# vasabi-root/gaus-slam

Measured on AMD Instinct MI355X. Metric: fwd+bwd frames/sec @ 640x480, 500k Gaussians, higher is better.
Workload: dtype f32

## Files before the change

### gaus_slam_amd/_lib.py

```python
import ctypes as C
import os

from . import _host, build as _build

ALLOC_FN = _host.ALLOC_FN

EXPORTS = ["gs2d_forward", "gs2d_backward", "gs2d_forward_posed", "gs2d_backward_posed", "gs2d_mark_visible", "sknn_dist2", "gs2d_geometry_bytes",
           "gs2d_image_bytes", "gs2d_binning_bytes", "gs2d_geometry_layout", "gs2d_binning_layout",
           "gs2d_image_layout", "gs2d_last_error", "gs2d_build_info", "gs2d_stage_timing_enable",
           "gs2d_stage_timing_read", "gs2d_slam_loss", "gs2d_adam_step", "gs2d_pose_quat", "gs2d_backward_staged", "gs2d_set_deterministic",
           "gs2d_get_deterministic", "gs2d_set_reference_binning", "gs2d_get_reference_binning", "gs2d_set_launch_ahead", "gs2d_get_launch_ahead", "gs2d_forward_batch",
           "gs2d_backward_batch", "gs2d_stage_timing_read_abs"]
MAX_FRAMES = 8


class FrameIO(C.Structure):
    _fields_ = [("geometry_alloc", ALLOC_FN), ("geometry_user", C.c_void_p), ("binning_alloc", ALLOC_FN),
                ("binning_user", C.c_void_p), ("image_alloc", ALLOC_FN), ("image_user", C.c_void_p),
                ("viewmatrix", C.c_void_p), ("projmatrix", C.c_void_p), ("cam_pos", C.c_void_p),
                ("out_color", C.c_void_p), ("out_others", C.c_void_p), ("radii", C.c_void_p)]


class FrameGrad(C.Structure):
    _fields_ = [("viewmatrix", C.c_void_p), ("projmatrix", C.c_void_p), ("campos", C.c_void_p), ("tan_fovx", C.c_float),
                ("tan_fovy", C.c_float), ("radii", C.c_void_p), ("geom_buffer", C.c_void_p), ("binning_buffer", C.c_void_p),
                ("img_buffer", C.c_void_p), ("num_rendered", C.c_int), ("dL_dpix", C.c_void_p), ("dL_depths", C.c_void_p),
                ("dL_dmean2D", C.c_void_p), ("dL_dnormal", C.c_void_p), ("dL_dopacity", C.c_void_p), ("dL_dcolor", C.c_void_p),
# ... 27 lines not shown
    L.gs2d_backward_posed.restype = i
    L.gs2d_backward_posed.argtypes = L.gs2d_backward.argtypes[:-1] + [vp, vp, vp, vp]
    L.gs2d_backward_staged.restype = i
    L.gs2d_backward_staged.argtypes = [i, i, i] + L.gs2d_backward_posed.argtypes
    L.gs2d_forward_batch.restype = i
    L.gs2d_forward_batch.argtypes = [i, C.POINTER(FrameIO), i, i, i, vp, i, i, vp, vp, vp, vp, vp, f, vp, vp, i, i,
                                     C.POINTER(C.c_int), vp]
    L.gs2d_backward_batch.restype = i
    L.gs2d_backward_batch.argtypes = [i, C.POINTER(FrameGrad), i, i, i, i, vp, i, i, vp, vp, vp, vp, f, vp, vp, i, i, vp]
    L.gs2d_pose_quat.restype = i
    L.gs2d_pose_quat.argtypes = [vp, vp, vp]
    L.gs2d_mark_visible.restype = i
    L.gs2d_mark_visible.argtypes = [i, vp, vp, vp, vp, vp]
    L.sknn_dist2.restype = i
    L.sknn_dist2.argtypes = [i, vp, vp, ALLOC_FN, vp, vp]
    for n in ("gs2d_geometry_bytes", "gs2d_binning_bytes"):
        getattr(L, n).restype = sz
        getattr(L, n).argtypes = [i]
    L.gs2d_image_bytes.restype = sz
    L.gs2d_image_bytes.argtypes = [i, i]
    L.gs2d_geometry_layout.argtypes = [i, C.POINTER(sz)]
    L.gs2d_binning_layout.argtypes = [i, C.POINTER(sz)]
    L.gs2d_image_layout.argtypes = [i, i, C.POINTER(sz)]
    L.gs2d_slam_loss.restype = i
    L.gs2d_slam_loss.argtypes = [i, i, i, vp, vp, vp, vp, f, f, f, f, f, i, i, f, f, f, vp, vp, vp, vp, vp, vp]
    L.gs2d_adam_step.restype = i
    L.gs2d_adam_step.argtypes = [i, vp, vp, C.c_double, C.c_double, f, i, C.c_ulonglong, vp, vp, vp, vp, vp]
    L.gs2d_set_deterministic.argtypes = [i]
    L.gs2d_get_deterministic.restype = i
    L.gs2d_set_reference_binning.argtypes = [i]
    L.gs2d_set_launch_ahead.argtypes = [i]
# ... 29 lines not shown
```

### gaus_slam_amd/csrc/gs2d_api.hip

```cpp
#include "gs2d_common.h"
#include "../../include/gs2d_rasterizer.h"

#include <stdio.h>
#include <stdlib.h>
#include <string.h>
#include <chrono>
#include <string>
#include <atomic>
#include <mutex>
#include <thread>
#if defined(__x86_64__) || defined(__i386__)
#include <immintrin.h>
#endif

namespace {

thread_local std::string g_err;

int fail(const char* what, hipError_t e)
{
    char buf[512];
    snprintf(buf, sizeof(buf), "gs2d: %s: %s", what, hipGetErrorString(e));
    g_err = buf;
    return -1;
// ... 162 lines not shown

size_t gs2d_geometry_bytes(int P) { return geom_layout(P).total; }
size_t gs2d_image_bytes(int width, int height) { return img_layout(width, height).total; }
size_t gs2d_binning_bytes(int R) { return bin_layout(R, g_deterministic.load() != 0).total; }

void gs2d_geometry_layout(int P, size_t o[5])
{
    const GeomLayout L = geom_layout(P);
    o[0] = L.depths; o[1] = L.tiles_touched; o[2] = L.point_offsets; o[3] = L.rec; o[4] = L.clamped;
}
void gs2d_binning_layout(int R, size_t o[2])
{
    const BinLayout L = bin_layout(R);
    o[0] = L.point_list; o[1] = L.keys;
}
void gs2d_image_layout(int width, int height, size_t o[2])
{
    const ImgLayout L = img_layout(width, height);
    o[0] = L.ranges; o[1] = L.pix;
}

}

namespace {

struct FwdShared {
    int P, D, M, width, height, use_sa, debug;
    const float* background;
    const float *means3D, *shs, *colors_precomp, *opacities, *scales, *rotations, *transMat_precomp;
    float scale_modifier;
// ... 171 lines not shown
            uint2* ranges = (uint2*)(img + IL.ranges);
            const int tile_bits = (int)higher_msb((uint32_t)(cam.gx * cam.gy));
            g_timer.begin(ST_SORT, s);
            gs2d::launch_bin_by_tile_dev(db, IL.tiles, tile_bits, ranges, s);
            const long long Rg = same_shape ? (long long)last.R : (long long)C0;
            const int cap_class = gs2d::tile_sort_capacity(Rg, IL.tiles);
            f.sort_cap = gs2d::gs2d_fused_sort_cap(cap_class);
            f.fused_sort = f.sort_cap > 0;
            if (!f.fused_sort) gs2d::launch_tile_depth_sort_dev(db, IL.tiles, ranges, cap_class, 0, s);
            g_timer.end(ST_SORT, s);
            GS2D_STAGE("bin by tile (count on the device)");
            f.ahead = true; f.cap = C0; f.det = false;
            f.bin = bin_pre;
            f.bf.ranges = ranges; f.bf.point_list = nullptr; f.bf.rec = (const float4*)(geom + GL.rec);
            f.bf.out_color = f.out_color; f.bf.out_others = f.out_others; f.bf.pix_state = (float*)(img + IL.pix);
            f.bf.hits = nullptr; f.bf.hits4 = nullptr; f.bf.zero = (float4*)(geom + GL.grad_rec);
            f.bf.keys = nullptr; f.bf.keys_alt = nullptr; f.bf.vals_alt = nullptr;
            f.bf.dev = db;
            return 0;
        }
    }
    if (!wait_total(f, s)) return fail_msg("num_rendered read-back failed");
    if (debug) GS2D_CHECK(hipStreamSynchronize(s), f.spec ? "duplicate" : "scan");
    const uint32_t num_rendered_u = *f.pinned;
    if (num_rendered_u == 0xFFFFFFFFu) return fail_msg("num_rendered read-back failed");
    if (num_rendered_u > 0x7fffffffu) return fail_msg("num_rendered overflows int32");
    const int R = (int)num_rendered_u;
    f.R = R;

    last.P = P; last.W = width; last.H = height; last.R = num_rendered_u;
    const bool reuse_pre = bin_pre && R <= C0;
// ... 39 lines not shown
        g_timer.begin(ST_RANGES, s);
        gs2d::launch_tile_ranges(R, keys, ranges, IL.tiles, s);
        g_timer.end(ST_RANGES, s);
        GS2D_STAGE("ranges");
    }
    f.sort_cap = one_pass && R > 0 ? gs2d::gs2d_fused_sort_cap(gs2d::tile_sort_capacity(R, IL.tiles)) : 0;
    f.fused_sort = f.sort_cap > 0;
    if (R > 0) {
        if (!f.fused_sort)
            gs2d::launch_tile_depth_sort(R, IL.tiles, ranges, keys, point_list, keys_alt, vals_alt, one_pass ? 1 : 0, debug ? 1 : 0, s);
        g_timer.end(ST_SORT, s);
        GS2D_STAGE("tile depth sort");
    }
    f.bf.ranges = ranges; f.bf.point_list = point_list; f.bf.rec = (const float4*)(geom + GL.rec);
    f.bf.out_color = f.out_color; f.bf.out_others = f.out_others; f.bf.pix_state = (float*)(img + IL.pix);
    f.bf.hits = (uint8_t*)(bin + BL.hits); f.bf.hits4 = (uint8_t*)(bin + BL.hits4);
    f.bf.zero = (float4*)(geom + GL.grad_rec);
    f.bf.keys = keys; f.bf.keys_alt = keys_alt; f.bf.vals_alt = vals_alt;
    f.bf.dev = gs2d::DevBin{nullptr, nullptr, 0u, 0};
    return 0;
}

int fwd_batch_fused(const FwdShared& c, FwdFrame* f, int K)
{
    const int debug = c.debug;
    hipStream_t s = c.s;
    const int P = c.P, width = c.width, height = c.height;
    const GeomLayout GL = geom_layout(P);
    const ImgLayout IL = img_layout(width, height);
    gs2d::PreFwdFrames pre;
    gs2d::BinFrames bin;
// ... 84 lines not shown
        f[k].bin_bytes = BL.total;
        gs2d::BinFrame& b = bin.f[k];
        b.capacity = (uint32_t)cap[k];
        b.total_host = nullptr;
        b.R = R;
        b.point_list = (uint32_t*)(bn + BL.point_list);
        b.keys = (uint64_t*)(bn + BL.keys);
        b.vals_alt = (uint32_t*)(bn + BL.vals_alt);
        b.keys_alt = (uint64_t*)(bn + BL.keys_alt);
        b.keys_unsorted = b.keys_alt; b.vals_unsorted = b.vals_alt;
        b.hist = (uint32_t*)(bn + BL.hist);
        b.ranges = (uint2*)(f[k].img + IL.ranges);
        gs2d::BlendFwdFrame& o = f[k].bf;
        o.ranges = b.ranges; o.point_list = b.point_list; o.rec = (const float4*)(f[k].geom + GL.rec);
        o.out_color = f[k].out_color; o.out_others = f[k].out_others; o.pix_state = (float*)(f[k].img + IL.pix);
        o.hits = (uint8_t*)(bn + BL.hits); o.hits4 = (uint8_t*)(bn + BL.hits4);
        o.zero = (float4*)(f[k].geom + GL.grad_rec);
        o.keys = b.keys; o.keys_alt = b.keys_alt; o.vals_alt = b.vals_alt;
        o.dev = gs2d::DevBin{nullptr, nullptr, 0u, 0};
    }
    if (debug) GS2D_CHECK(hipStreamSynchronize(s), "duplicate (batch)");
    for (int k = K; k < GS2D_MAX_BATCH; k++) bin.f[k] = bin.f[0];
    if (redo) {
        gs2d::launch_duplicate_batch(P, K, cam0.gx, bin, s);
        GS2D_STAGE("duplicate (batch, second launch)");
    }
    long long max_R = 0;
    bool any_empty = false;
    for (int k = 0; k < K; k++) { max_R = f[k].R > max_R ? f[k].R : max_R; any_empty = any_empty || f[k].R == 0; }
    const int sort_cap = any_empty ? 0 : gs2d::gs2d_fused_sort_cap(gs2d::tile_sort_capacity(max_R, IL.tiles));
    const bool fused_sort = sort_cap > 0;
// ... 195 lines not shown
    const bool pose_fast = (stages & 3) == 3 && g_begin == 0 && g_end == P && pose_Rt != nullptr && dL_dmean3D == nullptr && dL_dtransMat == nullptr &&
                           dL_dnormal == nullptr && dL_dsh == nullptr && shs == nullptr && scales != nullptr &&
                           rotations != nullptr && !det && !live_det;
    if (dL_dpose != nullptr && (stages & 1) != 0 && (R <= 0 || det))
        GS2D_CHECK(hipMemsetAsync(dL_dpose, 0, sizeof(float) * pose_floats, s), "memset dL_dpose");
    const GeomLayout GL = geom_layout(P);
    const BinLayout BL = bin_layout(R, det);
    if (known && (stages & 1) != 0 && R > 0 && BL.total > fr.bin_bytes)
        return fail_msg("binning chunk is smaller than the layout of this backward");
    const ImgLayout IL = img_layout(width, height);
    const float4* rec = (const float4*)(geom_buffer + GL.rec);
    const uint8_t* clamped = (const uint8_t*)(geom_buffer + GL.clamped);
    float* grad_rec = (float*)(geom_buffer + GL.grad_rec);
    const uint32_t* point_list = (const uint32_t*)(binning_buffer + BL.point_list);
    const uint8_t* hits = (const uint8_t*)(binning_buffer + BL.hits4);
    const uint2* ranges = (const uint2*)(img_buffer + IL.ranges);
    const float* pix_state = (const float*)(img_buffer + IL.pix);

    if ((stages & 1) != 0 && !det) {
        if (!(known && fr.clean))
            GS2D_CHECK(hipMemsetAsync(grad_rec, 0, sizeof(float) * GS2D_GRAD_FLOATS * (size_t)P, s), "memset grad_rec");
        if (R > 0) {
            g_timer.begin(ST_BLEND_BWD, s);
            const gs2d::BlendBwdFrame bf = {ranges, point_list, rec, pix_state, hits, dL_dpix, dL_depths, grad_rec, nullptr,
                                            (const uint16_t*)(binning_buffer + BL.hits), pose_fast ? grad_rec + 4 * (size_t)P : nullptr};
            gs2d::launch_blend_bwd(width, height, 1, &bf, background, use_sa, dL_dpose, pose_floats, s);
            g_timer.end(ST_BLEND_BWD, s);
            GS2D_STAGE("blend_bwd");
        }
    }
    if ((stages & 1) != 0 && det) {
        float* det_slots = (float*)(binning_buffer + BL.det_slots);
        uint32_t* det_inv = (uint32_t*)(binning_buffer + BL.det_inv);
        g_timer.begin(ST_BLEND_BWD, s);
        if (R > 0) {
            GS2D_CHECK(hipMemsetAsync(det_slots, 0, sizeof(float) * GS2D_GRAD_FLOATS * 4 * (size_t)R, s), "memset det_slots");
            const gs2d::BlendBwdFrame bf = {ranges, point_list, rec, pix_state, hits, dL_dpix, dL_depths, grad_rec, det_slots,
                                            (const uint16_t*)(binning_buffer + BL.hits), nullptr};
            gs2d::launch_blend_bwd(width, height, 1, &bf, background, use_sa, nullptr, 0, s);
        }
        gs2d::launch_det_reduce(P, R, width, height, ranges, point_list, (const ushort4*)(geom_buffer + GL.rect),
                                (const uint32_t*)(geom_buffer + GL.tiles_touched),
                                (const uint32_t*)(geom_buffer + GL.point_offsets), hits, det_inv, det_slots, grad_rec, s);
        g_timer.end(ST_BLEND_BWD, s);
        GS2D_STAGE("blend_bwd (deterministic)");
    }
    if ((stages & 2) != 0 && g_end > g_begin) {
        const float focal_y = height / (2.0f * tan_fovy);
        const float focal_x = width / (2.0f * tan_fovx);
        CamParams cam;
        cam.vm = viewmatrix; cam.pm = projmatrix; cam.campos = campos;
        cam.W = (int)(focal_x * tan_fovx * 2);
        cam.H = (int)(focal_y * tan_fovy * 2);
// ... 42 lines not shown
            if (R > 0 && rec.bin != (const void*)f.binning_buffer)
                return fail_msg("binning_buffer is not the chunk the forward of this geometry chunk was given");
            if (rec.det != 0) return fail_msg("gs2d_set_deterministic changed between this forward and its backward");
        }
        float* grad_rec = (float*)(f.geom_buffer + GL.grad_rec);
        if (!(known && rec.clean))
            GS2D_CHECK(hipMemsetAsync(grad_rec, 0, sizeof(float) * GS2D_GRAD_FLOATS * (size_t)P, s), "memset grad_rec");
        if (R > 0) {
            const BinLayout BL = bin_layout(R, false);
            if (known && BL.total > rec.bin_bytes) return fail_msg("binning chunk is smaller than the layout of this backward");
            gs2d::BlendBwdFrame& b = bf[nb++];
            b.ranges = (const uint2*)(f.img_buffer + IL.ranges);
            b.point_list = (const uint32_t*)(f.binning_buffer + BL.point_list);
            b.rec = (const float4*)(f.geom_buffer + GL.rec);
            b.pix_state = (const float*)(f.img_buffer + IL.pix);
            b.hits = (const uint8_t*)(f.binning_buffer + BL.hits4);
            b.dL_dpix = f.dL_dpix; b.dL_dothers = f.dL_depths; b.grad_rec = grad_rec; b.det_slots = nullptr; b.dense_m2d = nullptr;
            b.hits16 = (const uint16_t*)(f.binning_buffer + BL.hits);
        }
    }
    if (nb > 0) {
        g_timer.begin(ST_BLEND_BWD, s);
        gs2d::launch_blend_bwd(width, height, nb, bf, background, use_sa, nullptr, 0, s);
        g_timer.end(ST_BLEND_BWD, s);
        GS2D_STAGE("blend_bwd (batch)");
    }
    {
        gs2d::PreBwdFrames tab;
        for (int k = 0; k < K; k++) {
            const gs2d_frame_grad& f = fr[k];
            if (!f.dL_dmean2D || !f.dL_dopacity || !f.dL_dcolor || !f.dL_dmean3D || !f.dL_dscale || !f.dL_drot)
                return fail_msg("per-Gaussian gradient outputs are required for every frame of a batch");
            gs2d::PreBwdFrame& q = tab.f[k];
// ... 75 lines not shown
```

### gaus_slam_amd/csrc/gs2d_blend.hip

```cpp
#include "gs2d_common.h"
#ifndef GS2D_BWD_GROUPS
#define GS2D_BWD_GROUPS 4
#endif
#ifndef GS2D_BWD_POSE_GROUPS
#define GS2D_BWD_POSE_GROUPS 8
#endif
#define GS2D_HALFROW_BITS (GS2D_BWD_GROUPS == 8)
#ifndef GS2D_BWD_LANE_CLASH
#define GS2D_BWD_LANE_CLASH 1
#endif
#include "gs2d_cull.h"
#include "gs2d_tile_sort.h"
#include "gs2d_blend_dev.h"

#include <type_traits>

namespace {

__device__ __forceinline__ float fast_rcp(float x) { return __builtin_amdgcn_rcpf(x); }
__device__ __forceinline__ float fast_sqrt(float x) { return __builtin_amdgcn_sqrtf(x); }
__device__ __forceinline__ float fast_exp(float x) { return __builtin_amdgcn_exp2f(x * 1.44269504088896340736f); }
__device__ __forceinline__ float fast_exp_neg_half(float r) { return __builtin_amdgcn_exp2f(r * -0.72134752044448170368f); }
__device__ __forceinline__ float fast_exp_neg_quarter(float q) { return __builtin_amdgcn_exp2f(q * -0.36067376022224085184f); }

// ... 121 lines not shown
    if constexpr (BATCH) {
        const int frame = blockIdx.x / blocks_per_frame;
        local_block = blockIdx.x - frame * blocks_per_frame;
        fa = &args.f[frame];
    } else {
        fa = &args;
    }
    const uint2* __restrict__ ranges = fa->ranges;
    const uint32_t* __restrict__ point_list = fa->point_list;
    const float4* __restrict__ rec = fa->rec;
    float* __restrict__ out_color = fa->out_color;
    float* __restrict__ out_others = fa->out_others;
    float* __restrict__ pix_state = fa->pix_state;
    uint8_t* hits = fa->hits;
    uint8_t* hits4 = fa->hits4;
    float4* __restrict__ zero = fa->zero;
    uint64_t* sort_keys = fa->keys; uint64_t* sort_keys_alt = fa->keys_alt; uint32_t* sort_vals_alt = fa->vals_alt;
    uint32_t* sort_list = fa->point_list;
    if (fa->dev.base != nullptr) {
        const uint32_t Rd = *fa->dev.R_dev;
        if (Rd > fa->dev.cap) return;
        const BinLayout BL = bin_layout((int)Rd, fa->dev.det != 0, (int)fa->dev.cap);
        char* bb = fa->dev.base;
        sort_list = (uint32_t*)(bb + BL.point_list); point_list = sort_list;
        hits = (uint8_t*)(bb + BL.hits); hits4 = (uint8_t*)(bb + BL.hits4);
        sort_keys = (uint64_t*)(bb + BL.keys); sort_keys_alt = (uint64_t*)(bb + BL.keys_alt); sort_vals_alt = (uint32_t*)(bb + BL.vals_alt);
    }
    const int tile = xcd_tile(local_block, ntiles);
    if (tile < 0) { clear_share(zero, zero_n, local_block, blocks_per_frame); return; }
    if (sort_cap > 0) {
        if (sort_cap > GS2D_FUSED_SORT_CAP)
            tile_depth_sort_idx_body(tile, dyn_lds, reinterpret_cast<uint32_t (*)[256]>(dyn_lds + 2 * sort_cap), fa->ranges, sort_keys,
                                     sort_list, sort_keys_alt, sort_vals_alt, sort_cap, write_keys);
        else
            tile_depth_sort_body(tile, dyn_lds, reinterpret_cast<uint32_t (*)[256]>(dyn_lds + 4 * sort_cap), fa->ranges, sort_keys,
                                 sort_list, sort_keys_alt, sort_vals_alt, sort_cap, 1, write_keys);
        __builtin_amdgcn_fence(__ATOMIC_RELEASE, "workgroup");
        __syncthreads();
        __builtin_amdgcn_fence(__ATOMIC_ACQUIRE, "workgroup");
    }
    const int tx = tile % gx, ty = tile / gx;
    const int wave = threadIdx.x >> 6, lane = threadIdx.x & 63;
    FwdBatch& wb = batches[wave];
    const int qx0 = tx * GS2D_TILE + (wave & 1) * 8, qy0 = ty * GS2D_TILE + (wave >> 1) * 8;
    const int row = lane >> 2, li = lane & 3;
    const int lx = (row & 3) * 2 + (li & 1), ly = (row >> 2) * 2 + (li >> 1);
    const int px = qx0 + lx, py = qy0 + ly;
    const bool inside = px < W && py < H;
    const float pxf = (float)px, pyf = (float)py;
    const uint2 range = ranges[tile];
    const uint16_t* hits16 = reinterpret_cast<const uint16_t*>(hits);
    cull_tile_list(range, (float)(tx * GS2D_TILE), (float)(ty * GS2D_TILE), point_list, rec,
                   reinterpret_cast<uint64_t*>(hits), reinterpret_cast<uint32_t*>(hits4));
    __builtin_amdgcn_fence(__ATOMIC_RELEASE, "workgroup");
    __syncthreads();
    __builtin_amdgcn_fence(__ATOMIC_ACQUIRE, "workgroup");
    const float bg0 = bg[0], bg1 = bg[1], bg2 = bg[2];
    const uint8_t* qrow = wb.ql[row];
    if (lane < 4) wb.tail[lane] = 0x40404040u;
    if (lane == 4) wb.dead = make_float4(0.f, 0.f, 0.f, 0.f);

    float T = 1.0f, C0_ = 0.f, C1_ = 0.f, C2_ = 0.f, N0 = 0.f, N1 = 0.f, N2 = 0.f;
    float Dp = 0.f, M1 = 0.f, M2 = 0.f, D2 = 0.f, distortion = 0.f, median_depth = 0.f;
    uint32_t median_contributor = 0;
    uint32_t last_contributor = 0;
    uint64_t done_m = ballot64(!inside);
    GS2D_PROF_BEGIN();

    uint32_t next_chunk = range.x;
    uint32_t carry_base = 0, carry_tm = 0u, carry_id = 0u;
    bool carry = false;
    const uint32_t last_i = range.y > range.x ? range.y - 1u : range.x;
    uint32_t pf_tm = hits16[(size_t)min(next_chunk + lane, last_i) * 4 + wave];
// ... 26 lines not shown
            if (take) {
                wb.sid[slot] = id;
                wb.spos[slot] = cbase - range.x + lane + 1u;
                wb.tm[slot] = (uint16_t)tm;
            }
            if (fill + c > 64) { carry_tm = take ? 0u : tm; carry_id = id; carry_base = cbase; carry = true; fill = 64; break; }
            fill += c;
            if (fill == 64) break;
        }
        if (fill == 0) break;
        wave_lds_sync();
        if (lane < fill) {
            const float4* rp = rec + (size_t)wb.sid[lane] * GS2D_REC_F4;
            const float4 r0 = rp[0], r1 = rp[1], r2 = rp[2], r3 = rp[3];
            float4 r4 = rp[4];
            r4.w = __uint_as_float(wb.spos[lane]);
            wb.q(0)[lane] = r0; wb.q(1)[lane] = r1; wb.q(2)[lane] = r2; wb.q(3)[lane] = r3; wb.q(4)[lane] = r4;
        }
        if (fill == 0) break;
        wave_lds_sync();
        reinterpret_cast<uint4*>(&wb.ql[0][0])[lane] = make_uint4(0x40404040u, 0x40404040u, 0x40404040u, 0x40404040u);
        uint64_t dq = done_m;
        dq &= dq >> 1; dq &= dq >> 2; dq &= 0x1111111111111111ull;
        dq = (dq | (dq >> 3)) & 0x0303030303030303ull;
        dq = (dq | (dq >> 6)) & 0x000F000F000F000Full;
        dq = (dq | (dq >> 12)) & 0x000000FF000000FFull;
        const uint32_t done16 = (uint32_t)(dq | (dq >> 24)) & 0xFFFFu;
#ifdef GS2D_NO_DONE16
        const uint32_t nib = lane < fill ? (uint32_t)wb.tm[lane] : 0u; (void)done16;
#else
        const uint32_t nib = lane < fill ? (uint32_t)wb.tm[lane] & ~done16 : 0u;
#endif
        int trips = 0;
#pragma unroll
// ... 13 lines not shown
        {                                                                                                            \
            GS2D_PROF_TRIP();                                                                                        \
            const uint32_t contributor = __float_as_uint(C4.w);  \
            const bool live_ = contributor != 0u;                                                                    \
            N0_ = wb.q(0)[JN]; N1_ = wb.q(1)[JN]; N2_ = wb.q(2)[JN]; N3_ = wb.q(3)[JN];                              \
            N4_ = wb.q(4)[JN];                                                                                       \
            JNN = qrow[t + 2];                                                                                       \
            asm volatile("" : "+v"(JNN));  \
            float alpha, depth;                                                                                      \
            uint64_t ok_m;                                                                                           \
            fwd_eval(C0, C1, C2, pxf, pyf, alpha, depth, ok_m);                                                      \
            const float test_T = T * (1 - alpha);                                                                    \
            const uint64_t pass_m = ok_m & ballot64(live_) & ~done_m;                                                \
            const uint64_t stop_m = pass_m & ballot64(test_T < 0.0001f);                                             \
            done_m |= stop_m;                                                                                        \
            if (__builtin_amdgcn_inverse_ballot_w64(pass_m & ~stop_m)) {                                             \
                const float w = alpha * T;                                                                           \
                const uint64_t front_m = ballot64(T > 0.5f);                                                         \
                if (__builtin_amdgcn_inverse_ballot_w64(front_m)) { median_depth = depth; median_contributor = contributor; } \
                if (USE_SA) {                                                                \
                                          \
                    if (__builtin_amdgcn_inverse_ballot_w64(ballot64(Dp > 0) & ~front_m)) {                         \
                        const float exp_depth = median_depth;                                                        \
                        float exp_std = fmaf(fmaf(-2.0f * Dp, exp_depth, D2), fast_rcp(1 - T), exp_depth * exp_depth); \
                        exp_std = fmaxf(exp_std, 1e-7f);                                                             \
                        const float e = exp_depth - depth;                                                           \
                        const float conf = fast_exp_neg_quarter((e * e) * fast_rcp(exp_std));                        \
                        depth = fmaf(conf, depth, (1 - conf) * exp_depth);                                           \
                    }                                                                                                \
                    Dp = fmaf(depth, w, Dp);                                                                         \
                    D2 = fmaf(depth * depth, w, D2);                                                                 \
// ... 5 lines not shown
                    M1 = fmaf(m, w, M1);                                                                             \
                    M2 = fmaf(m * m, w, M2);                                                                         \
                }                                                                                                    \
                N0 = fmaf(C3.x, w, N0); N1 = fmaf(C3.y, w, N1); N2 = fmaf(C3.z, w, N2);                              \
                C0_ = fmaf(C3.w, w, C0_); C1_ = fmaf(C4.x, w, C1_); C2_ = fmaf(C4.y, w, C2_);                        \
                T = test_T;                                                                                          \
                last_contributor = contributor;                                                                      \
            }                                                                                                        \
            if (++t >= trips || ~done_m == 0ull) break;                                                              \
        }
        for (;;) {
            GS2D_FWD_STEP(a0, a1, a2, a3, a4, b0, b1, b2, b3, b4, jb, ja)
            GS2D_FWD_STEP(b0, b1, b2, b3, b4, a0, a1, a2, a3, a4, ja, jb)
        }
#undef GS2D_FWD_STEP
    }
    GS2D_PROF_END(0)
    if (inside) {
        const size_t HW = (size_t)H * W;
        const size_t pix = (size_t)W * py + px;
        out_color[pix] = fmaf(T, bg0, C0_);
        out_color[HW + pix] = fmaf(T, bg1, C1_);
        out_color[2 * HW + pix] = fmaf(T, bg2, C2_);
        const float dstd = fmaf(median_depth * median_depth, 1 - T, fmaf(-2.0f * median_depth, Dp, D2));
        out_others[pix] = Dp;
        out_others[HW + pix] = 1 - T;
        out_others[2 * HW + pix] = N0;
        out_others[3 * HW + pix] = N1;
        out_others[4 * HW + pix] = N2;
        out_others[5 * HW + pix] = median_depth;
// ... 254 lines not shown
    constexpr bool LANE_CLASH = !ROW_ACC && (NG == 8 || (GS2D_BWD_LANE_CLASH && !DET));
    __shared__ __attribute__((aligned(16))) unsigned char batch_mem[4 * BwdBatch::BYTES + GS2D_DEV_LDS_PAD];
    int local_block = blockIdx.x;
    const gs2d::BlendBwdFrame* fa;
    if constexpr (BATCH) {
        const int frame = blockIdx.x / blocks_per_frame;
        local_block = blockIdx.x - frame * blocks_per_frame;
        fa = &args.f[frame];
    } else {
        fa = &args;
    }
    const uint2* __restrict__ ranges = fa->ranges;
    const uint32_t* __restrict__ point_list = fa->point_list;
    const float4* __restrict__ rec = fa->rec;
    const float* __restrict__ pix_state = fa->pix_state;
    const uint8_t* __restrict__ hits = fa->hits;
    const uint16_t* __restrict__ hits16 = fa->hits16;
    const float* __restrict__ dL_dpix = fa->dL_dpix;
    const float* __restrict__ dL_dothers = fa->dL_dothers;
    float* __restrict__ grad_rec = fa->grad_rec;
    float* __restrict__ det_slots = fa->det_slots;
    float* __restrict__ dense_m2d = fa->dense_m2d;
    const int tile = xcd_tile(local_block, ntiles);
    if (tile < 0) return;
    const int tx = tile % gx, ty = tile / gx;
    const int wave = threadIdx.x >> 6, lane = threadIdx.x & 63;
    BwdBatch& wb = *reinterpret_cast<BwdBatch*>(batch_mem + wave * BwdBatch::BYTES);
    const int qx0 = tx * GS2D_TILE + (wave & 1) * 8, qy0 = ty * GS2D_TILE + (wave >> 1) * 8;
    const int row = lane >> 4, li = lane & 15;
    const int grp = NG == 8 ? lane >> 3 : row;
    const int grp8 = grp * 8;
    auto cull_bits = [&](uint32_t at) -> uint32_t {
        if (NG == 8 && !GS2D_HALFROW_BITS) return halfrows_from_groups_fast(hits16[(size_t)at * 4 + wave]);
        return hits[(size_t)at * 4 + wave];
    };
    const uint8_t* qrow = wb.ql[grp];
    const int px = qx0 + (row & 1) * 4 + (li & 3), py = qy0 + (row >> 1) * 4 + (li >> 2);
    const bool inside = px < W && py < H;
    const float pxf = (float)px, pyf = (float)py;
    const uint2 range = ranges[tile];
    const size_t HW = (size_t)H * W;
    const size_t pix = (size_t)W * py + px;
    const int flx = (row & 1) * 4 + (li & 3), fly = (row >> 1) * 4 + (li >> 2);
    const size_t si = (size_t)tile * GS2D_TILE_PIX + wave * 64 + ((fly >> 1) * 4 + (flx >> 1)) * 4 + (fly & 1) * 2 + (flx & 1);

    const float T_final = inside ? pix_state[PS_TFINAL * plane + si] : 0.f;
    float T = T_final;
    const uint32_t last_contributor = inside ? reinterpret_cast<const uint32_t*>(pix_state)[PS_LAST * plane + si] : 0u;
    const uint32_t median_contributor = inside ? reinterpret_cast<const uint32_t*>(pix_state)[PS_MEDC * plane + si] : 0u;
    float dpx0 = 0.f, dpx1 = 0.f, dpx2 = 0.f, dL_dreg = 0.f, dL_ddepth = 0.f, dL_daccum = 0.f;
// ... 58 lines not shown
        wave_lds_sync();
        uint32_t pf_tm = 0u, pf_id = 0u;
        if (chunk >= 0) {
            const uint32_t at = min(range.x + (uint32_t)chunk * 64u + lane, last_i);
            pf_tm = cull_bits(at);
            pf_id = point_list[at];
        }
        for (;;) {
            uint32_t tm, my_id;
            int cb;
            if (carry_chunk >= 0) { tm = carry_tm; my_id = carry_id; cb = carry_chunk; carry_chunk = -1; }
            else {
                if (chunk < 0) break;
                cb = chunk--;
                const int n = (int)min(64u, max_last - (uint32_t)cb * 64u);
                tm = lane < n ? ((NG == 8 || !GS2D_HALFROW_BITS) ? pf_tm : rows_from_halfrows(pf_tm)) : 0u;
                my_id = pf_id;
                const uint32_t nb = min(range.x + (uint32_t)max(chunk, 0) * 64u + lane, last_i);
                pf_tm = cull_bits(nb);
                pf_id = point_list[nb];
            }
            const uint64_t tb = ballot64(tm != 0u);
            const int c = __popcll(tb);
            if (c == 0) continue;
            const int slot = 64 - fill - c + rank_below(tb);
            const bool take = tm != 0u && slot >= 0;
            if (take) {
                wb.q(3)[slot].w = __uint_as_float(((uint32_t)cb * 64u + lane) | (NG == 8 ? (tm >> 4) << 28 : 0u));
                wb.pn[slot] = my_id | ((tm & 15u) << 28);
            }
            if (fill + c > 64) { carry_tm = take ? 0u : tm; carry_id = my_id; carry_chunk = cb; fill = 64; break; }
// ... 390 lines not shown
```

### gaus_slam_amd/csrc/gs2d_common.h

```cpp
#pragma once
#include <hip/hip_runtime.h>
#include <stddef.h>
#include <stdint.h>

#define GS2D_TILE 16
#define GS2D_TILE_PIX 256
#define GS2D_NEAR_N 0.2f
#define GS2D_FAR_N 100.0f
#define GS2D_FILTER_INV_SQ 100.0f

#define GS2D_REC_F4 5
#define GS2D_REC_FLOATS 20

#define GS2D_GRAD_FLOATS 20

enum { PS_TFINAL = 0, PS_M1, PS_M2, PS_MEDIAN, PS_STD, PS_LAST, PS_MEDC, PS_PLANES };

__host__ __device__ static inline size_t gs2d_align_up(size_t v, size_t a) { return (v + a - 1) / a * a; }

struct GeomLayout {
    size_t depths, tiles_touched, point_offsets, rec, clamped, scan_tmp, grad_rec, rect, total;
};
struct BinLayout {
    size_t point_list, hits, hits4, keys, vals_alt, keys_alt, hist, det_inv, det_slots, total;
    size_t hist_elems;
};
struct ImgLayout {
    size_t ranges, pix, total;
    int tiles;
};

#define GS2D_SCAN_ITEMS 1024
#define GS2D_SORT_ITEMS 2048
#ifndef GS2D_BIN_ITEMS
#define GS2D_BIN_ITEMS 4096
#endif
#define GS2D_BIN_MAX_TILES 4096

static inline GeomLayout geom_layout(int P)
// ... 24 lines not shown
        const size_t point_list = o; o = gs2d_align_up(o + 4 * n, 256);
        const size_t hits = o; o = gs2d_align_up(o + 8 * n, 256);
        const size_t hits4 = o; o = gs2d_align_up(o + 4 * n, 256);
        const size_t keys = o; o = gs2d_align_up(o + 8 * n, 256);
        const size_t nblk = (n + GS2D_SORT_ITEMS - 1) / GS2D_SORT_ITEMS;
        const size_t hist_elems = 256 * nblk;
        const size_t bin_elems = (size_t)GS2D_BIN_MAX_TILES * ((n + GS2D_BIN_ITEMS - 1) / GS2D_BIN_ITEMS);
        const size_t cap_elems = hist_elems > bin_elems ? hist_elems : bin_elems;
        const size_t scan_blk = (cap_elems + GS2D_SCAN_ITEMS - 1) / GS2D_SCAN_ITEMS;
        const size_t hist = o; o = gs2d_align_up(o + 4 * (cap_elems + scan_blk + 64 + GS2D_BIN_MAX_TILES), 256);
        size_t det_inv = o, det_slots = o;
        if (det) {
            o = gs2d_align_up(o + 4 * n, 256);
            det_slots = o; o = gs2d_align_up(o + 4 * (size_t)GS2D_GRAD_FLOATS * 4 * n, 256);
        }
        if (out) {
            out->point_list = point_list; out->hits = hits; out->hits4 = hits4; out->keys = keys; out->hist = hist;
            out->hist_elems = hist_elems; out->det_inv = det_inv; out->det_slots = det_slots;
        }
        return o;
    };
    (void)fixed_part(r, &L);
    size_t o = fixed_part(c, nullptr);
    L.vals_alt = o; o = gs2d_align_up(o + 4 * c, 256);
    L.keys_alt = o; o = gs2d_align_up(o + 8 * c, 256);
    L.total = o;
    return L;
}

static inline ImgLayout img_layout(int W, int H)
{
    ImgLayout L;
    const int gx = (W + GS2D_TILE - 1) / GS2D_TILE, gy = (H + GS2D_TILE - 1) / GS2D_TILE;
// ... 119 lines not shown
void launch_bin_sort_batch(int P, int K, int tiles, int gx, int nbits, BinFrames& tab, int write_keys, bool depth_sort, hipStream_t s);
int tile_sort_capacity(long long R, int tiles);
#define GS2D_FUSED_SORT_CAP 1536
#define GS2D_FUSED_SORT_CAP_IDX 3072
static inline int gs2d_fused_sort_cap(int cap_class)
{
    return cap_class <= GS2D_FUSED_SORT_CAP ? GS2D_FUSED_SORT_CAP : (cap_class <= GS2D_FUSED_SORT_CAP_IDX ? GS2D_FUSED_SORT_CAP_IDX : 0);
}
static inline size_t gs2d_fused_sort_lds(int sort_cap) { return (size_t)sort_cap * (sort_cap > GS2D_FUSED_SORT_CAP ? 8 : 16) + 4096; }

#define GS2D_MAX_BATCH 8
struct BlendFwdFrame {
    const uint2* ranges; uint32_t* point_list; const float4* rec;
    float* out_color; float* out_others; float* pix_state;
    uint8_t* hits; uint8_t* hits4;
    float4* zero;
    uint64_t* keys; uint64_t* keys_alt; uint32_t* vals_alt;
    DevBin dev;
};
struct BlendFwdBatch { BlendFwdFrame f[GS2D_MAX_BATCH]; };
struct BlendBwdFrame {
    const uint2* ranges; const uint32_t* point_list; const float4* rec; const float* pix_state; const uint8_t* hits;
    const float* dL_dpix; const float* dL_dothers; float* grad_rec;
    float* det_slots;
    const uint16_t* hits16;
    float* dense_m2d;
};
struct BlendBwdBatch { BlendBwdFrame f[GS2D_MAX_BATCH]; };
void launch_blend_fwd(int W, int H, int K, const BlendFwdFrame* frames, const float* bg, int use_sa, size_t zero_n, int sort_cap,
                      int write_keys, hipStream_t s);
void launch_blend_bwd(int W, int H, int K, const BlendBwdFrame* frames, const float* bg, int use_sa, float* clear12, int clear_n,
                      hipStream_t s);
void launch_det_reduce(int P, int R, int W, int H, const uint2* ranges, const uint32_t* point_list, const ushort4* rect,
                       const uint32_t* tiles_touched, const uint32_t* point_offsets, const uint8_t* hits,
                       uint32_t* inv, const float* det_slots, float* grad_rec, hipStream_t s);
}
```

### gaus_slam_amd/csrc/gs2d_cull.h

```cpp
#pragma once
#include "gs2d_common.h"

namespace {

__device__ __forceinline__ float cull_rcp(float x) { return __builtin_amdgcn_rcpf(x); }
__device__ __forceinline__ float cull_sqrt(float x) { return __builtin_amdgcn_sqrtf(x); }

__device__ __forceinline__ uint64_t place_group_row(uint32_t cm, int GY)
{
    const int sh = ((GY >> 2) * 2) * 16 + (GY & 3) * 4;
    return ((uint64_t)(cm & 0xFu) << sh) | ((uint64_t)((cm >> 4) & 0xFu) << (sh + 16));
}
__device__ __forceinline__ uint32_t interval_groups(float lo, float hi, float o)
{
    const float fa = ceilf((lo - o - 1.f) * 0.5f), fb = floorf((hi - o) * 0.5f);
    const int a = (int)fminf(fmaxf(fa, 0.f), 8.f);
    const int b = (int)fminf(fmaxf(fb, -1.f), 7.f);
    const uint32_t run = ((2u << b) - 1u) & ~((1u << a) - 1u);
    return (fb == fb && fa == fa) ? (b < 0 ? 0u : run) : 0xFFu;
}

__device__ __forceinline__ uint64_t splat_touch_mask64(const float4 q0, const float4 q1, const float4 q2, float rho_max,
                                                       float tx0, float ty0)
{
// ... 35 lines not shown
        }
        const float fa = ceilf((lo + (7.5f - 1.f - 1e-3f)) * 0.5f), fb = floorf((hi + (7.5f + 1e-3f)) * 0.5f);
        const int a = (int)fminf(fmaxf(fa, 0.f), 8.f);
        const int b = (int)fminf(fmaxf(fb, -1.f), 7.f);
        uint32_t cm = (b < 0) ? 0u : (((2u << b) - 1u) & ~((1u << a) - 1u));
        cm |= ((lp_rows >> GY) & 1u) ? lp_cols : 0u;
        m |= place_group_row(cm, GY);
    }
    return m;
}

__device__ __forceinline__ uint32_t rows_from_groups(uint32_t g16)
{
    return ((g16 & 0x0033u) ? 1u : 0u) | ((g16 & 0x00CCu) ? 2u : 0u) | ((g16 & 0x3300u) ? 4u : 0u) | ((g16 & 0xCC00u) ? 8u : 0u);
}
__device__ __forceinline__ uint32_t halfrows_from_groups(uint32_t g16)
{
    return ((g16 & 0x0003u) ? 0x01u : 0u) | ((g16 & 0x0030u) ? 0x02u : 0u) | ((g16 & 0x000Cu) ? 0x04u : 0u) | ((g16 & 0x00C0u) ? 0x08u : 0u) |
           ((g16 & 0x0300u) ? 0x10u : 0u) | ((g16 & 0x3000u) ? 0x20u : 0u) | ((g16 & 0x0C00u) ? 0x40u : 0u) | ((g16 & 0xC000u) ? 0x80u : 0u);
}
__device__ __forceinline__ uint32_t halfrows_from_groups_fast(uint32_t g16)
{
    uint32_t x = (g16 | (g16 >> 1)) & 0x5555u;
    x = (x | (x >> 1)) & 0x3333u;
    x = (x | (x >> 2)) & 0x0F0Fu;
    x = (x | (x >> 4)) & 0x00FFu;
    return (x & 0x99u) | ((x & 0x22u) << 1) | ((x & 0x44u) >> 1);
}
__device__ __forceinline__ uint32_t rows_from_halfrows(uint32_t h8)
{
    const uint32_t t = h8 | (h8 >> 1);
    return (t & 1u) | ((t >> 1) & 2u) | ((t >> 2) & 4u) | ((t >> 3) & 8u);
}

#ifndef GS2D_CULL_T
#define GS2D_CULL_T 256
#endif
__device__ __forceinline__ void cull_tile_list(const uint2 range, float tx0, float ty0, const uint32_t* __restrict__ point_list,
                                               const float4* __restrict__ rec, uint64_t* __restrict__ hits,
                                               uint32_t* __restrict__ hits4)
{
    uint32_t i = range.x + threadIdx.x;
    if (i >= range.y) return;
    const uint32_t last = range.y - 1;
    uint32_t id_next = point_list[min(i + GS2D_CULL_T, last)];
    const float4* rp = rec + (size_t)point_list[i] * GS2D_REC_F4;
    float4 r0 = rp[0], r1 = rp[1], r2 = rp[2];
    float rho_max = reinterpret_cast<const float*>(rp)[18];
    for (;;) {
        const uint32_t id_next2 = point_list[min(i + 2 * GS2D_CULL_T, last)];
        const float4* np = rec + (size_t)id_next * GS2D_REC_F4;
        const float4 n0 = np[0], n1 = np[1], n2 = np[2];
        const float nrho = reinterpret_cast<const float*>(np)[18];
        const uint64_t m64 = splat_touch_mask64(r0, r1, r2, rho_max, tx0, ty0);
        hits[i] = m64;
#if GS2D_HALFROW_BITS
        hits4[i] = halfrows_from_groups((uint32_t)m64 & 0xFFFFu) | (halfrows_from_groups((uint32_t)(m64 >> 16) & 0xFFFFu) << 8) |
                   (halfrows_from_groups((uint32_t)(m64 >> 32) & 0xFFFFu) << 16) | (halfrows_from_groups((uint32_t)(m64 >> 48)) << 24);
#else
        hits4[i] = rows_from_groups((uint32_t)m64 & 0xFFFFu) | (rows_from_groups((uint32_t)(m64 >> 16) & 0xFFFFu) << 8) |
                   (rows_from_groups((uint32_t)(m64 >> 32) & 0xFFFFu) << 16) | (rows_from_groups((uint32_t)(m64 >> 48)) << 24);
#endif
        i += GS2D_CULL_T;
        if (i >= range.y) break;
        r0 = n0; r1 = n1; r2 = n2; rho_max = nrho; id_next = id_next2;
    }
}

}
```

### include/gs2d_rasterizer.h

```cpp
#ifndef GS2D_RASTERIZER_H
#define GS2D_RASTERIZER_H

#include <stddef.h>
#include <stdint.h>

#ifdef __cplusplus
extern "C" {
#endif

typedef void* (*gs2d_alloc_fn)(void* user, size_t bytes);

int gs2d_forward(
    gs2d_alloc_fn geometry_alloc, void* geometry_user,
    gs2d_alloc_fn binning_alloc, void* binning_user,
    gs2d_alloc_fn image_alloc, void* image_user,
    int P, int D, int M,
    const float* background,
    int width, int height,
    const float* means3D,
    const float* shs,
    const float* colors_precomp,
    const float* opacities,
    const float* scales,
    float scale_modifier,
// ... 118 lines not shown
                   double* workspace , float* loss_out ,
                   float* dL_dcolor, float* dL_dallmap, const float* upstream ,
                   void* stream);

#define GS2D_ADAM_MAX_GROUPS 8
int gs2d_adam_step(int n_groups, const unsigned long long* group_end, const float* group_lr, double beta1, double beta2,
                   float eps, int step, unsigned long long n, float* param, const float* grad, float* exp_avg,
                   float* exp_avg_sq, void* stream);

size_t gs2d_geometry_bytes(int P);
size_t gs2d_image_bytes(int width, int height);
size_t gs2d_binning_bytes(int R);

void gs2d_geometry_layout(int P, size_t offsets[5]);
void gs2d_binning_layout(int R, size_t offsets[2]);
void gs2d_image_layout(int width, int height, size_t offsets[2]);

void gs2d_stage_timing_enable(int on);
int gs2d_stage_timing_read(float ms[9]);
int gs2d_stage_timing_read_abs(float ms[18]);

const char* gs2d_last_error(void);
const char* gs2d_build_info(void);

#ifdef __cplusplus
}
#endif
#endif
```

Measured before the change: 2316.

## Record per-halfrow contributor masks in forward blend to prune backward work

The forward blend kernel now records, per Gaussian entry and wave, which half-row pixel groups actually contributed (passed the alpha test before termination), using wave-scope atomic ORs into LDS and writing the result to a new contrib buffer in the binning allocation. The backward blend uses these contributor masks in place of the geometric touch masks (hits4/hits16), so it can skip Gaussians that overlap a region but were culled by alpha or early termination. This adds atomics and an extra byte write per entry in the forward pass and more binning memory, and the forward loop no longer breaks early when fill is zero.

Result: faster. 2371, median of 6 (+2.4%).

```diff
diff --git a/gaus_slam_amd/_lib.py b/gaus_slam_amd/_lib.py
--- a/gaus_slam_amd/_lib.py
+++ b/gaus_slam_amd/_lib.py
@@ -10,7 +10,7 @@
            "gs2d_image_layout", "gs2d_last_error", "gs2d_build_info", "gs2d_stage_timing_enable",
            "gs2d_stage_timing_read", "gs2d_slam_loss", "gs2d_adam_step", "gs2d_pose_quat", "gs2d_backward_staged", "gs2d_set_deterministic",
            "gs2d_get_deterministic", "gs2d_set_reference_binning", "gs2d_get_reference_binning", "gs2d_set_launch_ahead", "gs2d_get_launch_ahead", "gs2d_forward_batch",
-           "gs2d_backward_batch", "gs2d_stage_timing_read_abs"]
+           "gs2d_backward_batch", "gs2d_stage_timing_read_abs", "gs2d_binning_contrib_offset"]
 MAX_FRAMES = 8
 
 
@@ -68,7 +68,7 @@
     L.gs2d_mark_visible.argtypes = [i, vp, vp, vp, vp, vp]
     L.sknn_dist2.restype = i
     L.sknn_dist2.argtypes = [i, vp, vp, ALLOC_FN, vp, vp]
-    for n in ("gs2d_geometry_bytes", "gs2d_binning_bytes"):
+    for n in ("gs2d_geometry_bytes", "gs2d_binning_bytes", "gs2d_binning_contrib_offset"):
         getattr(L, n).restype = sz
         getattr(L, n).argtypes = [i]
     L.gs2d_image_bytes.restype = sz
diff --git a/gaus_slam_amd/csrc/gs2d_api.hip b/gaus_slam_amd/csrc/gs2d_api.hip
--- a/gaus_slam_amd/csrc/gs2d_api.hip
+++ b/gaus_slam_amd/csrc/gs2d_api.hip
@@ -200,6 +200,7 @@
     const BinLayout L = bin_layout(R);
     o[0] = L.point_list; o[1] = L.keys;
 }
+size_t gs2d_binning_contrib_offset(int R) { return bin_layout(R, g_deterministic.load() != 0).contrib; }
 void gs2d_image_layout(int width, int height, size_t o[2])
 {
     const ImgLayout L = img_layout(width, height);
@@ -401,7 +402,7 @@
             f.bin = bin_pre;
             f.bf.ranges = ranges; f.bf.point_list = nullptr; f.bf.rec = (const float4*)(geom + GL.rec);
             f.bf.out_color = f.out_color; f.bf.out_others = f.out_others; f.bf.pix_state = (float*)(img + IL.pix);
-            f.bf.hits = nullptr; f.bf.hits4 = nullptr; f.bf.zero = (float4*)(geom + GL.grad_rec);
+            f.bf.hits = nullptr; f.bf.hits4 = nullptr; f.bf.contrib = nullptr; f.bf.zero = (float4*)(geom + GL.grad_rec);
             f.bf.keys = nullptr; f.bf.keys_alt = nullptr; f.bf.vals_alt = nullptr;
             f.bf.dev = db;
             return 0;
@@ -471,7 +472,7 @@
     }
     f.bf.ranges = ranges; f.bf.point_list = point_list; f.bf.rec = (const float4*)(geom + GL.rec);
     f.bf.out_color = f.out_color; f.bf.out_others = f.out_others; f.bf.pix_state = (float*)(img + IL.pix);
-    f.bf.hits = (uint8_t*)(bin + BL.hits); f.bf.hits4 = (uint8_t*)(bin + BL.hits4);
+    f.bf.hits = (uint8_t*)(bin + BL.hits); f.bf.hits4 = (uint8_t*)(bin + BL.hits4); f.bf.contrib = (uint8_t*)(bin + BL.contrib);
     f.bf.zero = (float4*)(geom + GL.grad_rec);
     f.bf.keys = keys; f.bf.keys_alt = keys_alt; f.bf.vals_alt = vals_alt;
     f.bf.dev = gs2d::DevBin{nullptr, nullptr, 0u, 0};
@@ -586,7 +587,7 @@
         gs2d::BlendFwdFrame& o = f[k].bf;
         o.ranges = b.ranges; o.point_list = b.point_list; o.rec = (const float4*)(f[k].geom + GL.rec);
         o.out_color = f[k].out_color; o.out_others = f[k].out_others; o.pix_state = (float*)(f[k].img + IL.pix);
-        o.hits = (uint8_t*)(bn + BL.hits); o.hits4 = (uint8_t*)(bn + BL.hits4);
+        o.hits = (uint8_t*)(bn + BL.hits); o.hits4 = (uint8_t*)(bn + BL.hits4); o.contrib = (uint8_t*)(bn + BL.contrib);
         o.zero = (float4*)(f[k].geom + GL.grad_rec);
         o.keys = b.keys; o.keys_alt = b.keys_alt; o.vals_alt = b.vals_alt;
         o.dev = gs2d::DevBin{nullptr, nullptr, 0u, 0};
@@ -812,6 +813,7 @@
     float* grad_rec = (float*)(geom_buffer + GL.grad_rec);
     const uint32_t* point_list = (const uint32_t*)(binning_buffer + BL.point_list);
     const uint8_t* hits = (const uint8_t*)(binning_buffer + BL.hits4);
+    const uint8_t* contrib = (const uint8_t*)(binning_buffer + BL.contrib);
     const uint2* ranges = (const uint2*)(img_buffer + IL.ranges);
     const float* pix_state = (const float*)(img_buffer + IL.pix);
 
@@ -820,8 +822,8 @@
             GS2D_CHECK(hipMemsetAsync(grad_rec, 0, sizeof(float) * GS2D_GRAD_FLOATS * (size_t)P, s), "memset grad_rec");
         if (R > 0) {
             g_timer.begin(ST_BLEND_BWD, s);
-            const gs2d::BlendBwdFrame bf = {ranges, point_list, rec, pix_state, hits, dL_dpix, dL_depths, grad_rec, nullptr,
-                                            (const uint16_t*)(binning_buffer + BL.hits), pose_fast ? grad_rec + 4 * (size_t)P : nullptr};
+            const gs2d::BlendBwdFrame bf = {ranges, point_list, rec, pix_state, contrib, dL_dpix, dL_depths, grad_rec, nullptr,
+                                            pose_fast ? grad_rec + 4 * (size_t)P : nullptr};
             gs2d::launch_blend_bwd(width, height, 1, &bf, background, use_sa, dL_dpose, pose_floats, s);
             g_timer.end(ST_BLEND_BWD, s);
             GS2D_STAGE("blend_bwd");
@@ -833,8 +835,7 @@
         g_timer.begin(ST_BLEND_BWD, s);
         if (R > 0) {
             GS2D_CHECK(hipMemsetAsync(det_slots, 0, sizeof(float) * GS2D_GRAD_FLOATS * 4 * (size_t)R, s), "memset det_slots");
-            const gs2d::BlendBwdFrame bf = {ranges, point_list, rec, pix_state, hits, dL_dpix, dL_depths, grad_rec, det_slots,
-                                            (const uint16_t*)(binning_buffer + BL.hits), nullptr};
+            const gs2d::BlendBwdFrame bf = {ranges, point_list, rec, pix_state, contrib, dL_dpix, dL_depths, grad_rec, det_slots, nullptr};
             gs2d::launch_blend_bwd(width, height, 1, &bf, background, use_sa, nullptr, 0, s);
         }
         gs2d::launch_det_reduce(P, R, width, height, ranges, point_list, (const ushort4*)(geom_buffer + GL.rect),
@@ -907,9 +908,8 @@
             b.point_list = (const uint32_t*)(f.binning_buffer + BL.point_list);
             b.rec = (const float4*)(f.geom_buffer + GL.rec);
             b.pix_state = (const float*)(f.img_buffer + IL.pix);
-            b.hits = (const uint8_t*)(f.binning_buffer + BL.hits4);
+            b.contrib = (const uint8_t*)(f.binning_buffer + BL.contrib);
             b.dL_dpix = f.dL_dpix; b.dL_dothers = f.dL_depths; b.grad_rec = grad_rec; b.det_slots = nullptr; b.dense_m2d = nullptr;
-            b.hits16 = (const uint16_t*)(f.binning_buffer + BL.hits);
         }
     }
     if (nb > 0) {
diff --git a/gaus_slam_amd/csrc/gs2d_blend.hip b/gaus_slam_amd/csrc/gs2d_blend.hip
--- a/gaus_slam_amd/csrc/gs2d_blend.hip
+++ b/gaus_slam_amd/csrc/gs2d_blend.hip
@@ -5,7 +5,6 @@
 #ifndef GS2D_BWD_POSE_GROUPS
 #define GS2D_BWD_POSE_GROUPS 8
 #endif
-#define GS2D_HALFROW_BITS (GS2D_BWD_GROUPS == 8)
 #ifndef GS2D_BWD_LANE_CLASH
 #define GS2D_BWD_LANE_CLASH 1
 #endif
@@ -159,6 +158,7 @@
     float* __restrict__ pix_state = fa->pix_state;
     uint8_t* hits = fa->hits;
     uint8_t* hits4 = fa->hits4;
+    uint8_t* contrib = fa->contrib;
     float4* __restrict__ zero = fa->zero;
     uint64_t* sort_keys = fa->keys; uint64_t* sort_keys_alt = fa->keys_alt; uint32_t* sort_vals_alt = fa->vals_alt;
     uint32_t* sort_list = fa->point_list;
@@ -168,7 +168,7 @@
         const BinLayout BL = bin_layout((int)Rd, fa->dev.det != 0, (int)fa->dev.cap);
         char* bb = fa->dev.base;
         sort_list = (uint32_t*)(bb + BL.point_list); point_list = sort_list;
-        hits = (uint8_t*)(bb + BL.hits); hits4 = (uint8_t*)(bb + BL.hits4);
+        hits = (uint8_t*)(bb + BL.hits); hits4 = (uint8_t*)(bb + BL.hits4); contrib = (uint8_t*)(bb + BL.contrib);
         sort_keys = (uint64_t*)(bb + BL.keys); sort_keys_alt = (uint64_t*)(bb + BL.keys_alt); sort_vals_alt = (uint32_t*)(bb + BL.vals_alt);
     }
     const int tile = xcd_tile(local_block, ntiles);
@@ -196,12 +196,13 @@
     const uint2 range = ranges[tile];
     const uint16_t* hits16 = reinterpret_cast<const uint16_t*>(hits);
     cull_tile_list(range, (float)(tx * GS2D_TILE), (float)(ty * GS2D_TILE), point_list, rec,
-                   reinterpret_cast<uint64_t*>(hits), reinterpret_cast<uint32_t*>(hits4));
+                   reinterpret_cast<uint64_t*>(hits), reinterpret_cast<uint32_t*>(hits4), reinterpret_cast<uint32_t*>(contrib));
     __builtin_amdgcn_fence(__ATOMIC_RELEASE, "workgroup");
     __syncthreads();
     __builtin_amdgcn_fence(__ATOMIC_ACQUIRE, "workgroup");
     const float bg0 = bg[0], bg1 = bg[1], bg2 = bg[2];
     const uint8_t* qrow = wb.ql[row];
+    const uint32_t my_halfrow = halfrow_bit_of_group(row);
     if (lane < 4) wb.tail[lane] = 0x40404040u;
     if (lane == 4) wb.dead = make_float4(0.f, 0.f, 0.f, 0.f);
 
@@ -258,10 +259,11 @@
             const float4* rp = rec + (size_t)wb.sid[lane] * GS2D_REC_F4;
             const float4 r0 = rp[0], r1 = rp[1], r2 = rp[2], r3 = rp[3];
             float4 r4 = rp[4];
+            r4.z = __uint_as_float((uint32_t)lane);
             r4.w = __uint_as_float(wb.spos[lane]);
             wb.q(0)[lane] = r0; wb.q(1)[lane] = r1; wb.q(2)[lane] = r2; wb.q(3)[lane] = r3; wb.q(4)[lane] = r4;
         }
-        if (fill == 0) break;
+        wb.sid[lane] = 0u;
         wave_lds_sync();
         reinterpret_cast<uint4*>(&wb.ql[0][0])[lane] = make_uint4(0x40404040u, 0x40404040u, 0x40404040u, 0x40404040u);
         uint64_t dq = done_m;
@@ -305,7 +307,13 @@
             const uint64_t pass_m = ok_m & ballot64(live_) & ~done_m;                                                \
             const uint64_t stop_m = pass_m & ballot64(test_T < 0.0001f);                                             \
             done_m |= stop_m;                                                                                        \
-            if (__builtin_amdgcn_inverse_ballot_w64(pass_m & ~stop_m)) {                                             \
+            const uint64_t comp_m = pass_m & ~stop_m;                       \
+                                                                                   \
+            uint64_t quad_m = comp_m | (comp_m >> 1);                                                                \
+            quad_m = (quad_m | (quad_m >> 2)) & 0x1111111111111111ull;                                               \
+            if (__builtin_amdgcn_inverse_ballot_w64(quad_m))                                                         \
+                __hip_atomic_fetch_or(&wb.sid[__float_as_uint(C4.z)], my_halfrow, __ATOMIC_RELAXED, __HIP_MEMORY_SCOPE_WAVEFRONT); \
+            if (__builtin_amdgcn_inverse_ballot_w64(comp_m)) {                                                       \
                 const float w = alpha * T;                                                                           \
                 const uint64_t front_m = ballot64(T > 0.5f);                                                         \
                 if (__builtin_amdgcn_inverse_ballot_w64(front_m)) { median_depth = depth; median_contributor = contributor; } \
@@ -341,6 +349,8 @@
             GS2D_FWD_STEP(b0, b1, b2, b3, b4, a0, a1, a2, a3, a4, ja, jb)
         }
 #undef GS2D_FWD_STEP
+        wave_lds_sync();
+        if (lane < fill) contrib[(size_t)(range.x + wb.spos[lane] - 1u) * 4 + wave] = (uint8_t)wb.sid[lane];
     }
     GS2D_PROF_END(0)
     if (inside) {
@@ -625,8 +635,7 @@
     const uint32_t* __restrict__ point_list = fa->point_list;
     const float4* __restrict__ rec = fa->rec;
     const float* __restrict__ pix_state = fa->pix_state;
-    const uint8_t* __restrict__ hits = fa->hits;
-    const uint16_t* __restrict__ hits16 = fa->hits16;
+    const uint8_t* __restrict__ contrib = fa->contrib;
     const float* __restrict__ dL_dpix = fa->dL_dpix;
     const float* __restrict__ dL_dothers = fa->dL_dothers;
     float* __restrict__ grad_rec = fa->grad_rec;
@@ -641,10 +650,7 @@
     const int row = lane >> 4, li = lane & 15;
     const int grp = NG == 8 ? lane >> 3 : row;
     const int grp8 = grp * 8;
-    auto cull_bits = [&](uint32_t at) -> uint32_t {
-        if (NG == 8 && !GS2D_HALFROW_BITS) return halfrows_from_groups_fast(hits16[(size_t)at * 4 + wave]);
-        return hits[(size_t)at * 4 + wave];
-    };
+    auto cull_bits = [&](uint32_t at) -> uint32_t { return contrib[(size_t)at * 4 + wave]; };
     const uint8_t* qrow = wb.ql[grp];
     const int px = qx0 + (row & 1) * 4 + (li & 3), py = qy0 + (row >> 1) * 4 + (li >> 2);
     const bool inside = px < W && py < H;
@@ -733,7 +739,7 @@
                 if (chunk < 0) break;
                 cb = chunk--;
                 const int n = (int)min(64u, max_last - (uint32_t)cb * 64u);
-                tm = lane < n ? ((NG == 8 || !GS2D_HALFROW_BITS) ? pf_tm : rows_from_halfrows(pf_tm)) : 0u;
+                tm = lane < n ? (NG == 8 ? pf_tm : rows_from_halfrows(pf_tm)) : 0u;
                 my_id = pf_id;
                 const uint32_t nb = min(range.x + (uint32_t)max(chunk, 0) * 64u + lane, last_i);
                 pf_tm = cull_bits(nb);
diff --git a/gaus_slam_amd/csrc/gs2d_common.h b/gaus_slam_amd/csrc/gs2d_common.h
--- a/gaus_slam_amd/csrc/gs2d_common.h
+++ b/gaus_slam_amd/csrc/gs2d_common.h
@@ -22,7 +22,7 @@
     size_t depths, tiles_touched, point_offsets, rec, clamped, scan_tmp, grad_rec, rect, total;
 };
 struct BinLayout {
-    size_t point_list, hits, hits4, keys, vals_alt, keys_alt, hist, det_inv, det_slots, total;
+    size_t point_list, hits, hits4, keys, vals_alt, keys_alt, hist, det_inv, det_slots, contrib, total;
     size_t hist_elems;
 };
 struct ImgLayout {
@@ -77,9 +77,10 @@
             o = gs2d_align_up(o + 4 * n, 256);
             det_slots = o; o = gs2d_align_up(o + 4 * (size_t)GS2D_GRAD_FLOATS * 4 * n, 256);
         }
+        const size_t contrib = o; o = gs2d_align_up(o + 4 * n, 256);
         if (out) {
             out->point_list = point_list; out->hits = hits; out->hits4 = hits4; out->keys = keys; out->hist = hist;
-            out->hist_elems = hist_elems; out->det_inv = det_inv; out->det_slots = det_slots;
+            out->hist_elems = hist_elems; out->det_inv = det_inv; out->det_slots = det_slots; out->contrib = contrib;
         }
         return o;
     };
@@ -229,16 +230,17 @@
     const uint2* ranges; uint32_t* point_list; const float4* rec;
     float* out_color; float* out_others; float* pix_state;
     uint8_t* hits; uint8_t* hits4;
+    uint8_t* contrib;
     float4* zero;
     uint64_t* keys; uint64_t* keys_alt; uint32_t* vals_alt;
     DevBin dev;
 };
 struct BlendFwdBatch { BlendFwdFrame f[GS2D_MAX_BATCH]; };
 struct BlendBwdFrame {
-    const uint2* ranges; const uint32_t* point_list; const float4* rec; const float* pix_state; const uint8_t* hits;
+    const uint2* ranges; const uint32_t* point_list; const float4* rec; const float* pix_state;
+    const uint8_t* contrib;
     const float* dL_dpix; const float* dL_dothers; float* grad_rec;
     float* det_slots;
-    const uint16_t* hits16;
     float* dense_m2d;
 };
 struct BlendBwdBatch { BlendBwdFrame f[GS2D_MAX_BATCH]; };
diff --git a/gaus_slam_amd/csrc/gs2d_cull.h b/gaus_slam_amd/csrc/gs2d_cull.h
--- a/gaus_slam_amd/csrc/gs2d_cull.h
+++ b/gaus_slam_amd/csrc/gs2d_cull.h
@@ -73,18 +73,10 @@
 {
     return ((g16 & 0x0033u) ? 1u : 0u) | ((g16 & 0x00CCu) ? 2u : 0u) | ((g16 & 0x3300u) ? 4u : 0u) | ((g16 & 0xCC00u) ? 8u : 0u);
 }
-__device__ __forceinline__ uint32_t halfrows_from_groups(uint32_t g16)
+__device__ __forceinline__ uint32_t halfrow_bit_of_group(int g)
 {
-    return ((g16 & 0x0003u) ? 0x01u : 0u) | ((g16 & 0x0030u) ? 0x02u : 0u) | ((g16 & 0x000Cu) ? 0x04u : 0u) | ((g16 & 0x00C0u) ? 0x08u : 0u) |
-           ((g16 & 0x0300u) ? 0x10u : 0u) | ((g16 & 0x3000u) ? 0x20u : 0u) | ((g16 & 0x0C00u) ? 0x40u : 0u) | ((g16 & 0xC000u) ? 0x80u : 0u);
-}
-__device__ __forceinline__ uint32_t halfrows_from_groups_fast(uint32_t g16)
-{
-    uint32_t x = (g16 | (g16 >> 1)) & 0x5555u;
-    x = (x | (x >> 1)) & 0x3333u;
-    x = (x | (x >> 2)) & 0x0F0Fu;
-    x = (x | (x >> 4)) & 0x00FFu;
-    return (x & 0x99u) | ((x & 0x22u) << 1) | ((x & 0x44u) >> 1);
+    const int gx = g & 3, gy = g >> 2;
+    return 1u << (4 * (gy >> 1) + 2 * (gx >> 1) + (gy & 1));
 }
 __device__ __forceinline__ uint32_t rows_from_halfrows(uint32_t h8)
 {
@@ -97,7 +89,7 @@
 #endif
 __device__ __forceinline__ void cull_tile_list(const uint2 range, float tx0, float ty0, const uint32_t* __restrict__ point_list,
                                                const float4* __restrict__ rec, uint64_t* __restrict__ hits,
-                                               uint32_t* __restrict__ hits4)
+                                               uint32_t* __restrict__ hits4, uint32_t* __restrict__ contrib)
 {
     uint32_t i = range.x + threadIdx.x;
     if (i >= range.y) return;
@@ -113,13 +105,9 @@
         const float nrho = reinterpret_cast<const float*>(np)[18];
         const uint64_t m64 = splat_touch_mask64(r0, r1, r2, rho_max, tx0, ty0);
         hits[i] = m64;
-#if GS2D_HALFROW_BITS
-        hits4[i] = halfrows_from_groups((uint32_t)m64 & 0xFFFFu) | (halfrows_from_groups((uint32_t)(m64 >> 16) & 0xFFFFu) << 8) |
-                   (halfrows_from_groups((uint32_t)(m64 >> 32) & 0xFFFFu) << 16) | (halfrows_from_groups((uint32_t)(m64 >> 48)) << 24);
-#else
         hits4[i] = rows_from_groups((uint32_t)m64 & 0xFFFFu) | (rows_from_groups((uint32_t)(m64 >> 16) & 0xFFFFu) << 8) |
                    (rows_from_groups((uint32_t)(m64 >> 32) & 0xFFFFu) << 16) | (rows_from_groups((uint32_t)(m64 >> 48)) << 24);
-#endif
+        contrib[i] = 0u;
         i += GS2D_CULL_T;
         if (i >= range.y) break;
         r0 = n0; r1 = n1; r2 = n2; rho_max = nrho; id_next = id_next2;
diff --git a/include/gs2d_rasterizer.h b/include/gs2d_rasterizer.h
--- a/include/gs2d_rasterizer.h
+++ b/include/gs2d_rasterizer.h
@@ -156,6 +156,7 @@
 
 void gs2d_geometry_layout(int P, size_t offsets[5]);
 void gs2d_binning_layout(int R, size_t offsets[2]);
+size_t gs2d_binning_contrib_offset(int R);
 void gs2d_image_layout(int width, int height, size_t offsets[2]);
 
 void gs2d_stage_timing_enable(int on);
```
